# anassinator/pddp

Hardware: AMD Instinct MI355X
Metric: pddp_iterations_per_sec (higher is better)
Workload: dtype f32; 1 GPU; BASELINE.json configs[1]: cartpole n=4 m=1, known-dynamics iLQR, horizon=100, batch=4096 trajectories per GPU, bounds +-10 (eig-clamp + BoxQP branch), 10 line-search alphas; batch_per_gpu=4096, horizon=100, alphas=10, launch_form=10 rounds per launch, rounds_per_launch=10, backward_kernel_variant=0

## Files before the change

pddp_amd/csrc/accept.hpp:

```cpp
#pragma once

#include "pddp_common.hpp"

namespace pddp {

template <typename T>
struct AcceptArgs {
  int B, N, n, m, A;
  const T* Zc;
  const T* Uc;
  const T* Jc;
  const T* gains;
  const int32_t* bwd_status;
  double tol, max_reg;
  int n_iterations;
  T* Z;
  T* U;
  T* gains_acc;
  T* J_opt;
  double* mu;
  double* delta;
  int32_t* state;
  int32_t* iter;
  uint8_t* active;
  uint8_t* fresh;
  int32_t* n_live;
};

constexpr double kMuMin = 1e-6;
constexpr double kDelta0 = 2.0;

constexpr int kAcceptThreads = 64;
constexpr int kMaxAlphas = 16;
constexpr int kLiveShards = 256;


template <typename T>
struct AcceptIn {
  int bstat, iter;
  double mu, delta;
  T J_opt;
};
template <typename T>
PDDP_DEV AcceptIn<T> accept_load(const AcceptArgs<T>& a, int b) {
  AcceptIn<T> in;
  in.bstat = a.bwd_status[b];
  in.mu = a.mu[b];
  in.delta = a.delta[b];
  in.J_opt = a.J_opt[b];
  in.iter = a.iter[b];
  return in;
}

template <typename T>
PDDP_DEV int argmin_first(const T* J, int A, T& Jm_out) {
  int amin = 0;
  T Jm = J[0];
#pragma unroll
  for (int i = 1; i < kMaxAlphas; ++i) {
    const bool take = (i < A) && (Jm == Jm) && (J[i] < Jm || J[i] != J[i]);
    amin = take ? i : amin;
    Jm = take ? J[i] : Jm;
  }
  Jm_out = Jm;
  return amin;
}

template <typename T>
PDDP_DEV int accept_decide(const AcceptArgs<T>& a, int b, const AcceptIn<T>& in,
                           int amin, T J_new, bool& fresh_out) {
  int amin_out = -1;
  double mu = in.mu, delta = in.delta;
  int st;
  bool increase = false;
  if (in.bstat != 0) {
    increase = true;
    st = PDDP_STATE_NOT_PD;
  } else {
    const T J_opt = in.J_opt;
    if (J_new < J_opt) {
      amin_out = amin;
      delta = (delta < 1.0 ? delta : 1.0) / kDelta0;
      mu *= delta;
      if (mu <= kMuMin) mu = 0.0;
      const T rel = abs_(J_opt - J_new) / J_opt;
      st = (rel < (T)a.tol) ? PDDP_STATE_CONVERGED : PDDP_STATE_ACCEPTED;
      a.J_opt[b] = J_new;
    } else {
      increase = true;
      st = PDDP_STATE_REJECTED;
    }
  }
  if (increase) {
    delta = (delta > 1.0 ? delta : 1.0) * kDelta0;
    mu = (kMuMin > mu * delta) ? kMuMin : mu * delta;
    if (mu >= a.max_reg) st = PDDP_STATE_MAX_REG;
  }
  a.mu[b] = mu;
  a.delta[b] = delta;
  a.state[b] = st;
  uint8_t act = 0, fr = 0;
  if (st == PDDP_STATE_NOT_PD || st == PDDP_STATE_REJECTED) {
    act = 1;
  } else if (st == PDDP_STATE_ACCEPTED) {
    if (in.iter < a.n_iterations) {
      a.iter[b] = in.iter + 1;
      act = 1;
      fr = 1;
    }
  }
  a.active[b] = act;
  a.fresh[b] = fr;
  if (act && a.n_live != nullptr)
    atomicAdd(a.n_live + (b & (kLiveShards - 1)), 1);
  fresh_out = fr != 0;
  return amin_out;
}

}
```

pddp_amd/csrc/line_search_lds.hpp:

```cpp
#pragma once

#include <type_traits>
#include "models.hpp"
#include "problem_args.hpp"
#include "accept.hpp"
#include "riccati_n4.hpp"

namespace pddp {

template <typename T>
PDDP_DEV void group_copy(T* dst, const T* src, int count, int l16) {
  constexpr int kDeep = 8;
  for (int o0 = l16; o0 < count; o0 += 16 * kDeep) {
    T tmp[kDeep];
#pragma unroll
    for (int r = 0; r < kDeep; ++r) {
      const int o = o0 + 16 * r;
      tmp[r] = src[o < count ? o : 0];
    }
#pragma unroll
    for (int r = 0; r < kDeep; ++r) {
      const int o = o0 + 16 * r;
      if (o < count) dst[o] = tmp[r];
    }
  }
}

PDDP_DEV void store4(float* p, float a, float b, float c, float d) {
  *reinterpret_cast<float4*>(p) = make_float4(a, b, c, d);
}
PDDP_DEV void store4(double* p, double a, double b, double c, double d) {
  *reinterpret_cast<double2*>(p) = make_double2(a, b);
  *reinterpret_cast<double2*>(p + 2) = make_double2(c, d);
}

template <typename T, int n, int m>
PDDP_DEV void control_law(const T* z, const T* zr, const T* gr, const T* us,
                          T alpha, const T* umin, const T* umax, T* un) {
#pragma unroll
  for (int r = 0; r < m; ++r) {
    T s = T(0);
#pragma unroll
    for (int c = 0; c < n; ++c)
      s = n4::fma_(z[c] - zr[c], gr[m + r * n + c], s);
    const T du = n4::fma_(alpha, gr[r], s);
    const T v = us[r] + du;
    un[r] = clamp_nan(v, umin[r], umax[r]);
  }
}
PDDP_DEV float control_law_pk(f32x2 za, f32x2 zb, f32x2 zra, f32x2 zrb,
                              f32x2 g01, f32x2 g23, f32x2 g4u, float alpha,
                              float umin, float umax) {
  const f32x2 da = pk_sub(za, zra), db = pk_sub(zb, zrb);
  float s = n4::fma_(da.x, g01.y, 0.0f);
  s = n4::fma_(da.y, g23.x, s);
  s = n4::fma_(db.x, g23.y, s);
  s = n4::fma_(db.y, g4u.x, s);
  const float du = n4::fma_(alpha, g01.x, s);
  return clamp_nan(g4u.y + du, umin, umax);
}

#ifdef PDDP_WG_TIMELINE
__device__ long long g_search_timeline[1024][12];
#define PDDP_TLS(I)                                                           \
  do {                                                                        \
    if ((threadIdx.x & 255) == 0 && blockIdx.x < 1024)                        \
      g_search_timeline[blockIdx.x][(I) + 4 * (threadIdx.x >> 8)] =           \
          wall_clock64();                                                     \
  } while (0)
#define PDDP_TLS_AT(SLOT)                                                     \
  do {                                                                        \
    if (threadIdx.x == 0 && blockIdx.x < 1024)                                \
      g_search_timeline[blockIdx.x][SLOT] = wall_clock64();                   \
  } while (0)
#else
#define PDDP_TLS(I)
#define PDDP_TLS_AT(SLOT)
#endif

template <typename T>
struct PreStaged {
  const T* Zs;
  const T* Us;
  const T* Gs;
  int status;
  T J_opt;
  T* carry_rows = nullptr;
};
template <typename T, int MODEL, bool FUSED, int WPB, int H, unsigned QM,
          bool DENSE, bool PRE = false>
PDDP_DEV void line_search_lds_body(const ProblemT<T> P,
                                   const LineSearchArgs<T> a,
                                   const AcceptArgs<T> c, T* rec, T* Lout,
                                   unsigned char* smem_raw,
                                   const PreStaged<T> pre,
                                   const unsigned tid = threadIdx.x) {
  using D = ModelDims<MODEL>;
  constexpr int n = D::n, m = D::m;
  constexpr int GS = m + m * n;
  static_assert(H == 1 || (H == 2 && FUSED), "");
  static_assert(!DENSE || (FUSED && H == 1), "");
  static_assert(!PRE || (FUSED && H == 2 && !DENSE), "");
  constexpr int GST = PRE ? GS + m : GS;
  constexpr int UST = PRE ? GS + m : m;
  constexpr int kTailRows = DENSE ? 8 : 4;
  constexpr bool kPaired = PRE && MODEL == PDDP_MODEL_CARTPOLE &&
                           std::is_same<T, float>::value && GST == 6 &&
                           QM == kSparseMask<PDDP_MODEL_CARTPOLE>;
  __shared__ int sh_dec[WPB][4][2];
  const int lane = tid & (kWave - 1);
  const int wave_all = tid >> 6;
  const int wave = H == 1 ? wave_all : wave_all % WPB;
  const int hid = H == 1 ? 0 : wave_all / WPB;
  const int grp = lane >> 4, ai = lane & 15;
  const int N = a.N;
  const int per = DENSE ? N * GS : (N + 1) * n + N * m + N * GS;
  T* smem = reinterpret_cast<T*>(smem_raw) + (size_t)wave * 4 * per;
  const int b0 = (blockIdx.x * WPB + wave) * 4;
  PDDP_TLS(0);

  for (int g = 0; g < (PRE ? 0 : 4); ++g) {
    const int bg = b0 + g;
    if (bg >= a.B) break;
    if (H == 2 && (g & 1) != hid) continue;
    if (a.active != nullptr && a.active[bg] == 0) continue;
    T* dst = smem + (size_t)g * per;
    const T* zs = a.Z + (size_t)bg * (N + 1) * n;
    const T* us = a.U + (size_t)bg * N * m;
    const T* gs = a.gains + (size_t)bg * N * GS;
    if constexpr (DENSE) {
      for (int o = lane; o < N * GS; o += kWave) dst[o] = gs[o];
    } else {
      for (int o = lane; o < (N + 1) * n; o += kWave) dst[o] = zs[o];
      for (int o = lane; o < N * m; o += kWave) dst[(N + 1) * n + o] = us[o];
      for (int o = lane; o < N * GS; o += kWave)
        dst[(N + 1) * n + N * m + o] = gs[o];
    }
  }
  if constexpr (!PRE) __syncthreads();
  PDDP_TLS(1);

  const int b = b0 + grp;
  const bool exists = b < a.B;
  const int bc = exists ? b : a.B - 1;
  const bool attempted =
      exists && (a.active == nullptr || a.active[bc] != 0);
  const bool run =
      attempted && ai < a.A &&
      (PRE ? pre.status == 0
           : (a.bwd_status == nullptr || a.bwd_status[bc] == 0));
  if constexpr (!FUSED) {
    if (!run) return;
  }
  const bool bounded = a.u_min != nullptr && a.u_max != nullptr;
  T umin[m], umax[m];
#pragma unroll
  for (int r = 0; r < m; ++r) {
    umin[r] = bounded ? a.u_min[r] : -(T)__builtin_inff();
    umax[r] = bounded ? a.u_max[r] : (T)__builtin_inff();
  }
  const T* Zs = PRE ? pre.Zs
                    : DENSE ? a.Z + (size_t)bc * (N + 1) * n
                            : smem + (size_t)grp * per;
  const T* Us = PRE ? pre.Us
                    : DENSE ? a.U + (size_t)bc * N * m : Zs + (N + 1) * n;
  const T* Gs = PRE ? pre.Gs : DENSE ? smem + (size_t)grp * per : Us + N * m;
  const size_t zstep_c = (size_t)a.A * n, ustep_c = (size_t)a.A * m;
  AcceptIn<T> acc_in = {};
  if constexpr (FUSED) {
    if (attempted && ai == 0) {
      acc_in = accept_load(c, b);
      if constexpr (PRE) {
        acc_in.bstat = pre.status;
        acc_in.J_opt = pre.J_opt;
      }
    }
  }
  T Jmine = T(0);
  const bool nocand = FUSED && n <= 4 && Lout == nullptr && rec != nullptr &&
                      a.drop_candidates != 0 && N + 1 <= 16 * H * kTailRows;
  const bool store_uc = !(FUSED && n <= 6 && Lout == nullptr &&
                          rec != nullptr && N + 1 <= 16 * H * kTailRows);
  auto rollout = [&](T alpha, T* Zci, size_t zstep, T* Uci, size_t ustep,
                     auto cost) {
    if constexpr (kPaired) {
      typedef float V4_ __attribute__((ext_vector_type(4)));
      V4_ z4 = {Zs[0], Zs[1], Zs[2], Zs[3]};
      float J = 0.0f;
      auto step = [&](const int t) {
        const V4_ zr = *reinterpret_cast<const V4_*>(
            __builtin_assume_aligned(Zs + t * 4, 16));
        const f32x2* g2 = reinterpret_cast<const f32x2*>(
            __builtin_assume_aligned(Gs + t * 6, 8));
        const f32x2 g01 = g2[0], g23 = g2[1], g4u = g2[2];
        const f32x2 sc = sincos_pk(z4.z);
        __builtin_amdgcn_sched_barrier(0);
        __builtin_amdgcn_s_waitcnt(0xC07F);
        const float u = control_law_pk(z4.xy, z4.zw, zr.xy, zr.zw, g01, g23,
                                       g4u, alpha, umin[0], umax[0]);
#pragma unroll
        for (int j = 0; j < 4; ++j) Zci[(size_t)t * zstep + j] = z4[j];
        J += cartpole_cost_pk(P, z4.xy, sc, u);
        if constexpr (decltype(cost)::value) asm("" : "+v"(J));
        f32x2 na, nb;
        cartpole_dynamics_pk(P, z4.xy, z4.zw, sc, u, na, nb);
        z4 = V4_{na.x, na.y, nb.x, nb.y};
      };
      int t = 0;
      for (; t + 3 < N; t += 4) {
        step(t);
        step(t + 1);
        step(t + 2);
        step(t + 3);
      }
#pragma unroll 1
      for (; t < N; ++t) step(t);
      T z[n] = {z4.x, z4.y, z4.z, z4.w};
#pragma unroll
      for (int j = 0; j < n; ++j) Zci[(size_t)N * zstep + j] = z[j];
      const T lf =
          cost_value<T, MODEL>(P, z, nullptr, trig_of<T, MODEL>(z), true);
      return J + lf;
    }
    T z[n], zn[n], un[m];
#pragma unroll
    for (int j = 0; j < n; ++j) z[j] = Zs[j];
    T J = T(0);
    auto step = [&](const int t) {
      T zr[n], gr[GS], us[m];
      if constexpr (PRE && n == 4) {
        typedef T V4_ __attribute__((ext_vector_type(4)));
        const V4_ v = *reinterpret_cast<const V4_*>(
            __builtin_assume_aligned(Zs + t * 4, 16));
        zr[0] = v[0]; zr[1] = v[1]; zr[2] = v[2]; zr[3] = v[3];
      } else {
#pragma unroll
        for (int j = 0; j < n; ++j) zr[j] = Zs[t * n + j];
      }
      if constexpr (PRE && GST == 6) {
        typedef T V2_ __attribute__((ext_vector_type(2)));
        const V2_* g2 = reinterpret_cast<const V2_*>(
            __builtin_assume_aligned(Gs + t * 6, 8));
        const V2_ a0 = g2[0], a1 = g2[1], a2 = g2[2];
        gr[0] = a0[0]; gr[1] = a0[1]; gr[2] = a1[0]; gr[3] = a1[1];
        gr[4] = a2[0]; us[0] = a2[1];
      } else {
#pragma unroll
        for (int j = 0; j < GS; ++j) gr[j] = Gs[t * GST + j];
#pragma unroll
        for (int j = 0; j < m; ++j) us[j] = Us[t * UST + j];
      }
      const Trig<T, MODEL> tr = trig_of<T, MODEL>(z);
      __builtin_amdgcn_sched_barrier(0);
      if constexpr (PRE) __builtin_amdgcn_s_waitcnt(0xC07F);
      control_law<T, n, m>(z, zr, gr, us, alpha, umin, umax, un);
#pragma unroll
      for (int j = 0; j < n; ++j) Zci[(size_t)t * zstep + j] = z[j];
      if constexpr (!PRE) {
        if (store_uc) {
#pragma unroll
          for (int j = 0; j < m; ++j) Uci[(size_t)t * ustep + j] = un[j];
        }
      }
      J += cost_value<T, MODEL, QM>(P, z, un, tr, false);
      dynamics<T, MODEL, false>(P, z, un, tr, zn, nullptr, nullptr);
#pragma unroll
      for (int j = 0; j < n; ++j) z[j] = zn[j];
    };
    int t = 0;
    if constexpr (n <= 4) {
      for (; t + 3 < N; t += 4) {
        step(t);
        step(t + 1);
        step(t + 2);
        step(t + 3);
      }
    }
#pragma unroll 1
    for (; t < N; ++t) step(t);
#pragma unroll
    for (int j = 0; j < n; ++j) Zci[(size_t)N * zstep + j] = z[j];
    const T lf =
        cost_value<T, MODEL>(P, z, nullptr, trig_of<T, MODEL>(z), true);
    return J + lf;
  };
  if (run && hid == 0) {
    const T alpha = a.alphas[ai];
    const int idx = b * a.A + ai;
    const bool compact0 = FUSED && Lout == nullptr && rec != nullptr &&
                          ai == 0 && n <= 6 && N + 1 <= 16 * H * kTailRows;
    T* Zci = compact0 ? rec + (size_t)b * (N + 1) * n
                      : a.Zc + ((size_t)b * (N + 1) * a.A + ai) * n;
    T* Uci = a.Uc + ((size_t)b * N * a.A + ai) * m;
    const size_t zstep = compact0 ? (size_t)n : (nocand ? 0 : zstep_c);
    const size_t ustep = nocand ? 0 : ustep_c;
    Jmine = rollout(alpha, Zci, zstep, Uci, ustep, std::true_type{});
    a.Jc[idx] = Jmine;
  }
  PDDP_TLS(2);

  if constexpr (FUSED) {
    constexpr int kNone = 99;
    const T kInf = (T)__builtin_inff();
    const int nan_first =
        n4::group_min((run && Jmine != Jmine) ? ai : kNone);
    T Jf = (run && Jmine == Jmine) ? Jmine : kInf;
    {
      T y = n4::dpp<0x128>(Jf); Jf = y < Jf ? y : Jf;
      y = n4::dpp<0x12C>(Jf); Jf = y < Jf ? y : Jf;
      y = n4::dpp<(2 | (3 << 2) | (0 << 4) | (1 << 6))>(Jf); Jf = y < Jf ? y : Jf;
      y = n4::dpp<(1 | (0 << 2) | (3 << 4) | (2 << 6))>(Jf); Jf = y < Jf ? y : Jf;
    }
    const int min_first = n4::group_min((run && Jmine == Jf) ? ai : kNone);
    const int amin =
        nan_first != kNone ? nan_first : (min_first != kNone ? min_first : 0);
    const T J_new = nan_first != kNone ? (T)__builtin_nanf("") : Jf;

    int amin_out = -1, fresh_i = 0;
    if (attempted && ai == 0 && hid == 0) {
      bool fr;
      amin_out = accept_decide(c, b, acc_in, amin, J_new, fr);
      fresh_i = fr ? 1 : 0;
    }
    amin_out = __shfl(amin_out, lane & 48);
    fresh_i = __shfl(fresh_i, lane & 48);
    PDDP_TLS_AT(8);
    if constexpr (n <= 4) {
      if (nocand && hid == 0 && __any(amin_out > 0)) {
        if (amin_out > 0 && ai == amin_out)
          rollout(a.alphas[ai], rec + (size_t)b * (N + 1) * n, (size_t)n,
                  a.Uc + ((size_t)b * N * a.A + ai) * m, 0, std::false_type{});
      }
    }
    if constexpr (H == 1) {
      if (!__any(amin_out >= 0)) return;
      __builtin_amdgcn_fence(__ATOMIC_ACQ_REL, "workgroup");
    } else {
      if (hid == 0 && ai == 0) {
        sh_dec[wave][grp][0] = amin_out;
        sh_dec[wave][grp][1] = fresh_i;
      }
      __builtin_amdgcn_fence(__ATOMIC_ACQ_REL, "workgroup");
      __syncthreads();
      amin_out = sh_dec[wave][grp][0];
      fresh_i = sh_dec[wave][grp][1];
    }
    PDDP_TLS_AT(9);
    if (amin_out >= 0) {
      constexpr RecLayout lay(n, m);
      constexpr int S = lay.stride;
      const T* srcz = a.Zc + ((size_t)b * (N + 1) * a.A + amin_out) * n;
      const T* srcu = a.Uc + ((size_t)b * N * a.A + amin_out) * m;
      T* Zb = c.Z + (size_t)b * (N + 1) * n;
      T* Ub = c.U + (size_t)b * N * m;
      T* rec_b = rec + (size_t)b * (N + 1) * S;
      T* Ls = PRE ? nullptr : smem + (size_t)grp * per;
      const T* G = c.gains + (size_t)b * N * GS;
      T* Ga = c.gains_acc + (size_t)b * N * GS;
      T zc[n], uc[m];
      const int t_first = ai + 16 * hid;
      constexpr int KR = kTailRows;
      if (n <= 6 && Lout == nullptr && N + 1 <= 16 * H * KR) {
        T zz[KR][n], uu[KR][m];
        const bool from_rec = rec != nullptr && (amin_out == 0 || nocand);
        const T* cz = from_rec ? rec + (size_t)b * (N + 1) * n : srcz;
        const size_t czs = from_rec ? (size_t)n : zstep_c;
#pragma unroll
        for (int k = 0; k < KR; ++k) {
          const int t = t_first + 16 * H * k;
          const int tz = t <= N ? t : N;
#pragma unroll
          for (int j = 0; j < n; ++j) zz[k][j] = cz[(size_t)tz * czs + j];
        }
        const T* Gl = Gs;
        if constexpr (PRE) {
          for (int t = ai + 16 * hid; t < N; t += 16 * H) {
#pragma unroll
            for (int j = 0; j < GS; ++j) Ga[t * GS + j] = Gl[t * GST + j];
          }
        } else {
          constexpr int kDeep = 8;
          int o = ai + 16 * hid;
          for (; o + 16 * H * (kDeep - 1) < N * GS; o += 16 * H * kDeep) {
            T tmp[kDeep];
#pragma unroll
            for (int r = 0; r < kDeep; ++r) tmp[r] = Gl[o + 16 * H * r];
#pragma unroll
            for (int r = 0; r < kDeep; ++r) Ga[o + 16 * H * r] = tmp[r];
          }
          for (; o < N * GS; o += 16 * H) Ga[o] = Gl[o];
        }
        PDDP_TLS_AT(10);
        const T alpha_w = a.alphas[amin_out];
#pragma unroll
        for (int k = 0; k < KR; ++k) {
          const int t = t_first + 16 * H * k;
          const int tu = t < N ? t : 0;
          if constexpr (kPaired) {
            typedef float V4_ __attribute__((ext_vector_type(4)));
            const V4_ zr = *reinterpret_cast<const V4_*>(
                __builtin_assume_aligned(Zs + tu * 4, 16));
            const f32x2* g2 = reinterpret_cast<const f32x2*>(
                __builtin_assume_aligned(Gs + tu * 6, 8));
            uu[k][0] = control_law_pk(f32x2{zz[k][0], zz[k][1]},
                                      f32x2{zz[k][2], zz[k][3]}, zr.xy, zr.zw,
                                      g2[0], g2[1], g2[2], alpha_w, umin[0],
                                      umax[0]);
            continue;
          }
          T zr[n], gr[GS], us[m];
#pragma unroll
          for (int j = 0; j < n; ++j) zr[j] = Zs[tu * n + j];
#pragma unroll
          for (int j = 0; j < GS; ++j) gr[j] = Gs[tu * GST + j];
#pragma unroll
          for (int j = 0; j < m; ++j) us[j] = Us[tu * UST + j];
          control_law<T, n, m>(zz[k], zr, gr, us, alpha_w, umin, umax, uu[k]);
        }
#pragma unroll
        for (int k = 0; k < KR; ++k) {
          const int t = t_first + 16 * H * k;
          if (t <= N) {
#pragma unroll
            for (int j = 0; j < n; ++j) Zb[t * n + j] = zz[k][j];
          }
          if (t < N) {
#pragma unroll
            for (int j = 0; j < m; ++j) Ub[t * m + j] = uu[k][j];
          }
          if constexpr (PRE) {
            if (pre.carry_rows != nullptr && t <= N && N - t <= 16) {
              T* cr = pre.carry_rows + (N - t) * (n + m);
#pragma unroll
              for (int j = 0; j < n; ++j) cr[j] = zz[k][j];
              if (t < N) {
#pragma unroll
                for (int j = 0; j < m; ++j) cr[n + j] = uu[k][j];
              }
            }
          }
        }
      } else {
      {
        const int tz = t_first <= N ? t_first : N;
        const int tu = t_first < N ? t_first : 0;
#pragma unroll
        for (int j = 0; j < n; ++j) zc[j] = srcz[(size_t)tz * zstep_c + j];
#pragma unroll
        for (int j = 0; j < m; ++j) uc[j] = srcu[(size_t)tu * ustep_c + j];
      }
#pragma unroll 1
      for (int t = t_first; t <= N; t += 16 * H) {
        T zn_[n], un_[m];
        {
          const int t2 = t + 16 * H;
          const int tz = t2 <= N ? t2 : N, tu = t2 < N ? t2 : 0;
#pragma unroll
          for (int j = 0; j < n; ++j) zn_[j] = srcz[(size_t)tz * zstep_c + j];
#pragma unroll
          for (int j = 0; j < m; ++j) un_[j] = srcu[(size_t)tu * ustep_c + j];
        }
        const bool terminal = (t == N);
        T un[m];
#pragma unroll
        for (int j = 0; j < m; ++j) un[j] = terminal ? T(0) : uc[j];
#pragma unroll
        for (int j = 0; j < n; ++j) Zb[t * n + j] = zc[j];
        if (!terminal) {
#pragma unroll
          for (int j = 0; j < m; ++j) Ub[t * m + j] = un[j];
        }
        if (fresh_i && Lout != nullptr) {
          T w[S];
          const T l = record_of<T, MODEL>(P, zc, un, terminal, bounded, a.u_min,
                                         a.u_max, w);
          T* dst = rec_b + (size_t)t * S;
#pragma unroll
          for (int j = 0; j < S; j += 4)
            store4(dst + j, w[j], w[j + 1], w[j + 2], w[j + 3]);
          Lout[(size_t)b * (N + 1) + t] = l;
          Ls[t] = l;
        }
#pragma unroll
        for (int j = 0; j < n; ++j) zc[j] = zn_[j];
#pragma unroll
        for (int j = 0; j < m; ++j) uc[j] = un_[j];
      }
      if constexpr (H == 1) {
        group_copy(Ga, G, N * GS, ai);
      } else {
        const int half = (N * GS + 1) / 2;
        const int off = hid * half;
        const int cnt = hid == 0 ? half : N * GS - half;
        group_copy(Ga + off, G + off, cnt, ai);
      }
      }
      if constexpr (H == 1) {
        if (fresh_i && Lout != nullptr) {
          __builtin_amdgcn_fence(__ATOMIC_RELEASE, "wavefront");
          __builtin_amdgcn_wave_barrier();
          if (ai == 0) {
            T Jacc = T(0);
            for (int t = 0; t <= N; ++t) Jacc += Ls[t];
            c.J_opt[b] = Jacc;
            c.fresh[b] = 0;
          }
        }
      }
    }
    if constexpr (H == 2) {
      __syncthreads();
      if (!PRE && amin_out >= 0 && fresh_i && Lout != nullptr && hid == 0 &&
          ai == 0) {
        const T* Ls = smem + (size_t)grp * per;
        T Jacc = T(0);
        for (int t = 0; t <= N; ++t) Jacc += Ls[t];
        c.J_opt[b] = Jacc;
        c.fresh[b] = 0;
      }
    }
  }
  PDDP_TLS(3);
// ... 19 lines not shown
```

pddp_amd/csrc/riccati_n4_elem.hpp:

```cpp
#pragma once

#include <type_traits>
#include "models.hpp"
#include "riccati_n4_quad.hpp"

namespace pddp {

namespace n4d {
typedef float f32x4 __attribute__((ext_vector_type(4)));
PDDP_DEV int sgn(float x) { return __float_as_int(x); }
PDDP_DEV int splat(int w) {
  int r;
  asm("v_ashrrev_i32 %0, 31, %1" : "=v"(r) : "v"(w));
  return r;
}
PDDP_DEV float bsel(int mask, float a, float b) {
  float r;
  asm("v_bfi_b32 %0, %1, %2, %3" : "=v"(r) : "v"(mask), "v"(a), "v"(b));
  return r;
}

template <typename T>
struct GenArgs {
  const T* Z;
  const T* U;
  T* L;
  T* J_opt;
  uint8_t* fresh;
};
}

namespace n4e {

using n4::bperm;
using n4::dpp;
using n4::fma_;
using n4::group_sum;
using n4::kGain;
using n4::mul_nc;
using n4d::bsel;
using n4d::f32x4;
typedef float f32x2 __attribute__((ext_vector_type(2)));
typedef float f32x3 __attribute__((ext_vector_type(3)));
using n4d::GenArgs;
using n4d::sgn;
using n4d::splat;

constexpr int kWaves = 4;
constexpr int kTrajW = 4;
constexpr int kBlk = 16;
constexpr int kImg = 52;
constexpr int kRowStride = kBlk * kImg + 16;
constexpr int kImgBuf = kTrajW * kRowStride;
constexpr int kTermRow = 24;
constexpr int kTermSh = kTrajW * kTermRow;
constexpr int kPairLdsInl = kImgBuf;
constexpr int kPairLdsOvl = 2 * kImgBuf + kTermSh;

struct LsTableF {
  float v[n4::kLsSteps];
  constexpr LsTableF() : v() {
    for (int n = 0; n < n4::kLsSteps; ++n) v[n] = (float)n4::kLs.v[n];
  }
};
__device__ constexpr LsTableF kLsF{};
template <typename T>
PDDP_DEV const T* ls_table();
template <>
PDDP_DEV const float* ls_table<float>() { return kLsF.v; }
template <>
PDDP_DEV const double* ls_table<double>() { return n4::kLs.v; }
template <typename T>
struct Vec {
  typedef T v4 __attribute__((ext_vector_type(4)));
  typedef T v2 __attribute__((ext_vector_type(2)));
};

PDDP_DEV f32x2 lo_word(float a) {
  f32x2 r;
  r.x = a;
  return r;
}
PDDP_DEV f32x2 box_gaps(f32x2 lh, float x) {
  f32x2 d;
  asm("v_pk_add_f32 %0, %1, %2 op_sel_hi:[1,0] neg_lo:[0,1] neg_hi:[1,0]"
      : "=v"(d)
// ... 239 lines not shown
    } else {
      oddm = alive_m;
    }
    bool fail = false;
    if (__builtin_expect(oddm != 0, F32 ? 0 : 1)) {
      const bool take = (oddm & lane_bit) != 0;
      n4::QpClosed<T, true> qc;
      qc.solve(take ? kprev : T(0), take ? Quug : T(1), take ? Qu : T(0), lo_b,
               hi_b);
      T kx = qc.x;
      bool Kzero = !qc.free_;
      fail = qc.fail & take;
      const bool slow = qc.slow & take;
      if (__builtin_expect(__any(slow), 0)) {
        unsigned long long todo = __ballot(slow && l == 0);
        while (todo != 0) {
          const int src = __builtin_ctzll(todo);
          todo &= todo - 1;
          const n4::SlowQpOut<T> o = n4q::boxqp1_wave<T, true>(
              __shfl(kprev, src), __shfl(Quug, src), __shfl(Qu, src),
              __shfl(lo_b, src), __shfl(hi_b, src), ls_table<T>(), lane);
          const bool mine = (lane >> 4) == (src >> 4);
          kx = mine ? o.x : kx;
          Kzero = mine ? ((o.result_free & 1) == 0) : Kzero;
          fail = mine ? (o.result_free < 2) : fail;
        }
      }
      kt = take ? kx : kt;
      sK = take ? (Kzero ? T(0) : qc.inv) : sK;
    }
    if (fail) st = PDDP_BWD_BOXQP_FAILED;
  }
  return st;
}

#ifdef PDDP_ELEM_MARKS
__device__ long long g_elem_marks[8];
#define PDDP_EM_MARK(I) do { if (blockIdx.x == 0 && threadIdx.x == 0) g_elem_marks[I] = clock64(); } while (0)
#define PDDP_EM_ACC(I, T0) do { if (blockIdx.x == 0 && threadIdx.x == 0) g_elem_marks[I] += clock64() - (T0); } while (0)
#define PDDP_EM_NOW() clock64()
#else
#define PDDP_EM_MARK(I)
#define PDDP_EM_ACC(I, T0)
#define PDDP_EM_NOW() 0
#endif

#ifdef PDDP_WG_TIMELINE
__device__ long long g_elem_timeline[1024][12];
#define PDDP_TL(I)                                                            \
  do {                                                                        \
    if ((threadIdx.x & 255) == 0 && blockIdx.x < 1024)                        \
      g_elem_timeline[blockIdx.x][(I) + 4 * (threadIdx.x >> 8)] =             \
          wall_clock64();                                                     \
  } while (0)
#define PDDP_TL_HW(I)                                                         \
  do {                                                                        \
    if (threadIdx.x == 0 && blockIdx.x < 1024) {                              \
      g_elem_timeline[blockIdx.x][8] =                                        \
          __builtin_amdgcn_s_getreg(4 | (0 << 6) | (31 << 11));               \
      g_elem_timeline[blockIdx.x][9] =                                        \
          __builtin_amdgcn_s_getreg(20 | (0 << 6) | (3 << 11));               \
      g_elem_timeline[blockIdx.x][I] = clock64();                             \
    }                                                                         \
  } while (0)
#else
#define PDDP_TL(I)
#define PDDP_TL_HW(I)
#endif

struct RoundOut {
  const float* Zs;
  const float* Gs;
  const float* Us;
  int status;
  float J_opt;
  float* carry_rows;
};
constexpr int round_zu_stride(int N) { return 4 * (N + 1); }
constexpr int kCarryRows = kBlk + 1, kCarryW = 5;
constexpr int kCarryF = kTrajW * kCarryRows * kCarryW;
constexpr int kGainL = kGain + 1;
constexpr int round_gains_floats(int N) { return (kTrajW * N * kGainL + 3) & ~3; }

template <typename T, unsigned QM, bool OVL, bool ROUND, int BR = kBrEigBox>
PDDP_DEV bool elem_sweep_body(const RiccatiArgs<T>& a, const GenArgs<T>& gen,
                              const ProblemT<T>& prob, unsigned char* smem_raw,
                              RoundOut& ro,
                              const unsigned tid = threadIdx.x,
                              const int carry = -1) {
  static_assert(OVL || !ROUND, "");
  constexpr bool F32 = std::is_same<T, float>::value;
  static_assert(F32 || (!OVL && !ROUND), "");
  using V4 = typename Vec<T>::v4;
  using V2 = typename Vec<T>::v2;
  constexpr int MODEL = PDDP_MODEL_CARTPOLE;
  constexpr RecLayout lay(4, 1);
  constexpr bool BOUNDED = br_bounded(BR), CHOL = br_chol(BR);
  const int kPairLds = OVL ? kPairLdsOvl + (ROUND ? round_gains_floats(a.N) +
                                                        (carry >= 0 ? kCarryF : 0)
                                                  : 0)
                           : kPairLdsInl;
  const int lane = tid & (kWave - 1);
  const int wave = __builtin_amdgcn_readfirstlane((int)tid >> 6);
  const int pair = OVL ? (wave & (kWaves - 1)) : wave;
  const bool is_gen = OVL && wave >= kWaves;
  T* const img0 = reinterpret_cast<T*>(smem_raw) + pair * kPairLds;
  T* const term_w = OVL ? img0 + 2 * kImgBuf : img0;

  const int row = lane >> 4, l = lane & 15, i = l >> 2, j = l & 3;
  const int N = a.N;
  const int b0 = (blockIdx.x * kWaves + pair) * kTrajW;
  const int b = b0 + row;
  const bool exists = b < a.B;
  const int bc = exists ? b : a.B - 1;
  const T* Zg = gen.Z + (size_t)bc * (size_t)(N + 1) * 4;
  const T* Ug = gen.U + (size_t)bc * (size_t)N;
  const int nblk = (N + kBlk - 1) / kBlk;
  if (b0 >= a.B) return false;
  const bool counted = exists && (a.active == nullptr || a.active[bc] != 0);
  if (!__any(counted)) return false;
  PDDP_EM_MARK(0);
  PDDP_TL(0);
  PDDP_TL_HW(10);
  T umin = T(0), umax = T(0);
  if constexpr (BOUNDED) { umin = a.u_min[0]; umax = a.u_max[0]; }
  const int rbase = row * kRowStride;

  T zq[4], uq, Jacc = T(0), l_term = T(0);
  [[maybe_unused]] T* const carry_w =
      img0 + kPairLdsOvl + (ROUND ? round_gains_floats(N) : 0) +
      row * kCarryRows * kCarryW;
  if constexpr (ROUND) ro.carry_rows = carry >= 0 ? carry_w : nullptr;
  auto request = [&](int jb) {
    int tau = N - 1 - kBlk * jb - l;
    tau = tau < 0 ? 0 : tau;
    if constexpr (ROUND) {
      if (jb == 0 && carry == 0) {
        const T* cr = carry_w + (N - tau) * kCarryW;
        zq[0] = cr[0]; zq[1] = cr[1]; zq[2] = cr[2]; zq[3] = cr[3];
        uq = cr[4];
        return;
      }
    }
    const V4 v = *reinterpret_cast<const V4*>(Zg + 4 * tau);
    zq[0] = v[0]; zq[1] = v[1]; zq[2] = v[2]; zq[3] = v[3];
    uq = Ug[tau];
    if constexpr (ROUND) {
      if (jb == 0 && carry == 1 && N - tau <= kBlk) {
        T* cr = carry_w + (N - tau) * kCarryW;
        cr[0] = zq[0]; cr[1] = zq[1]; cr[2] = zq[2]; cr[3] = zq[3];
        cr[4] = uq;
      }
    }
  };
  auto terminal = [&]() {
    T zN[4];
    if (ROUND && carry == 0) {
      zN[0] = carry_w[0]; zN[1] = carry_w[1]; zN[2] = carry_w[2];
      zN[3] = carry_w[3];
    } else {
      const V4 zNv = *reinterpret_cast<const V4*>(Zg + 4 * N);
      zN[0] = zNv[0]; zN[1] = zNv[1]; zN[2] = zNv[2]; zN[3] = zNv[3];
      if (ROUND && carry == 1 && l == 0) {
        carry_w[0] = zN[0]; carry_w[1] = zN[1]; carry_w[2] = zN[2];
        carry_w[3] = zN[3];
      }
    }
    T lz[4], lzz[16], lu[1], luu[1];
    l_term = cost_derivs<T, MODEL>(prob, zN, nullptr, trig_of<T, MODEL>(zN),
                                   true, lz, lzz, lu, luu);
    T* scr = term_w + row * kTermRow;
    if (l == 0) {
#pragma unroll
      for (int k = 0; k < 16; k += 4)
        *reinterpret_cast<V4*>(scr + k) =
            V4{lzz[k], lzz[k + 1], lzz[k + 2], lzz[k + 3]};
      *reinterpret_cast<V4*>(scr + 16) = V4{lz[0], lz[1], lz[2], lz[3]};
      scr[20] = l_term;
      if (counted) gen.L[(size_t)bc * (size_t)(N + 1) + N] = l_term;
    }
  };
  auto pass = [&](int jb, T* buf) {
    const T z[4] = {zq[0], zq[1], zq[2], zq[3]};
    const T u = uq;
    if (jb + 1 < nblk) request(jb + 1);
    const int tau = N - 1 - kBlk * jb - l;
    T w[lay.stride];
    const T lc = record_of<T, MODEL, QM>(prob, z, &u, false, BOUNDED, a.u_min,
                                         a.u_max, w);
    T* dst = buf + rbase + l * kImg;
#pragma unroll
    for (int r = 0; r < 4; ++r)
      *reinterpret_cast<V4*>(dst + 4 * r) =
          V4{w[lay.oFz + ((r + 0) & 3) * 4 + r],
                w[lay.oFz + ((r + 1) & 3) * 4 + r],
                w[lay.oFz + ((r + 2) & 3) * 4 + r],
                w[lay.oFz + ((r + 3) & 3) * 4 + r]};
#pragma unroll
    for (int x = 0; x < 4; x += 2) {
      *reinterpret_cast<V4*>(dst + 16 + 2 * x) =
          V4{w[lay.oFu + x], w[lay.oLuz + x], w[lay.oFu + x + 1],
                w[lay.oLuz + x + 1]};
      *reinterpret_cast<V4*>(dst + 24 + 2 * x) =
          V4{w[lay.oFu + x], w[lay.oLz + x], w[lay.oFu + x + 1],
                w[lay.oLz + x + 1]};
    }
#pragma unroll
    for (int r = 0; r < 4; ++r)
      *reinterpret_cast<V4*>(dst + 32 + 4 * r) =
          V4{w[lay.oLzz + 4 * r], w[lay.oLzz + 4 * r + 1],
                w[lay.oLzz + 4 * r + 2], w[lay.oLzz + 4 * r + 3]};
    *reinterpret_cast<V4*>(dst + 48) =
        V4{w[lay.oLuu], w[lay.oLu], BOUNDED ? umin - w[lay.oU] : T(0),
           BOUNDED ? umax - w[lay.oU] : T(0)};
    if (tau >= 0) {
      if (counted) gen.L[(size_t)bc * (size_t)(N + 1) + tau] = lc;
      Jacc += lc;
    }
  };
  auto finish_costs = [&]() {
    const bool sums = counted && (gen.fresh == nullptr || gen.fresh[bc] != 0);
    const T Jrow = group_sum(Jacc) + (OVL ? term_w[row * kTermRow + 20] : l_term);
    if constexpr (ROUND) {
      const T Jold = gen.J_opt[bc];
      if (l == 0) term_w[row * kTermRow + 21] = sums ? Jrow : Jold;
    }
    if (sums && l == 0) {
      gen.J_opt[bc] = Jrow;
      if (gen.fresh != nullptr) gen.fresh[bc] = 0;
    }
  };
  [[maybe_unused]] T* const gains_w = img0 + kPairLdsOvl;
  auto flush_gains = [&](const T* ib, int t_top, int cnt) {
    const T* sg = ib + l * kImg + rbase;
    const V4 Kv = *reinterpret_cast<const V4*>(sg);
    const T kv = sg[4];
    if ((BR == kBrEigBox ? exists : counted) && l < cnt) {
      T* g = a.gains + ((size_t)bc * (size_t)N + (size_t)(t_top - l)) * kGain;
      g[0] = kv; g[1] = Kv[0]; g[2] = Kv[1]; g[3] = Kv[2]; g[4] = Kv[3];
      if constexpr (ROUND) {
        T* gl = gains_w + (row * N + (t_top - l)) * kGainL;
        gl[0] = kv; gl[1] = Kv[0]; gl[2] = Kv[1]; gl[3] = Kv[2]; gl[4] = Kv[3];
      }
    }
  };
  [[maybe_unused]] T* const zu_w =
      img0 + (nblk & 1) * kImgBuf + row * round_zu_stride(N);
  [[maybe_unused]] auto round_out = [&](int status_) {
    if constexpr (ROUND) {
      ro.Zs = zu_w;
      ro.Gs = gains_w + row * N * kGainL;
      ro.Us = ro.Gs + kGain;
      ro.status = status_;
      n4::lds_publish_barrier();
      ro.J_opt = term_w[row * kTermRow + 21];
    }
  };
  if constexpr (OVL) {
    if (is_gen) {
      request(0);
      pass(0, img0);
      PDDP_TL(1);
      n4::lds_publish_barrier();
      for (int jb = 1; jb < nblk; ++jb) {
        if (jb >= 2)
          flush_gains(img0 + (jb & 1) * kImgBuf, N - 1 - kBlk * (jb - 2), kBlk);
        pass(jb, img0 + (jb & 1) * kImgBuf);
        n4::lds_publish_barrier();
      }
      if (nblk >= 2)
        flush_gains(img0 + (nblk & 1) * kImgBuf, N - 1 - kBlk * (nblk - 2), kBlk);
      if constexpr (ROUND) {
        asm volatile("s_waitcnt lgkmcnt(0)" ::: "memory");
        constexpr int kCh = 8;
        V4 zc[kCh];
        T uc[kCh];
#pragma unroll
        for (int c = 0; c < kCh; ++c) {
          const int tz = l + 16 * c;
          zc[c] = *reinterpret_cast<const V4*>(Zg + 4 * (tz <= N ? tz : N));
          uc[c] = Ug[tz < N ? tz : 0];
        }
#pragma unroll
        for (int c = 0; c < kCh; ++c) {
          const int tz = l + 16 * c;
          if (tz <= N) *reinterpret_cast<V4*>(zu_w + 4 * tz) = zc[c];
          if (tz < N) gains_w[(row * N + tz) * kGainL + kGain] = uc[c];
        }
      }
      finish_costs();
      PDDP_TL(3);
      if constexpr (ROUND) round_out(PDDP_BWD_OK);
      return true;
    }
  }

  const T reg = (T)a.reg[bc];
  const int oA = rbase + 4 * i, oB = rbase + 4 * j, oL = rbase + 32 + l;
  const int oTi = rbase + 16 + 2 * i, oTj = rbase + 24 + 2 * j;
  const int tr_addr = ((lane & 48) | (j * 4 + i)) * 4;
  if constexpr (OVL) {
    __builtin_amdgcn_s_setprio(3);
    terminal();
    n4::lds_publish_barrier();
  } else {
    request(0);
    terminal();
    asm volatile("s_waitcnt lgkmcnt(0)" ::: "memory");
  }
  T V = term_w[row * kTermRow + l];
  T vc = term_w[row * kTermRow + 16 + j];

  struct Words {
    V4 Fs, Fq;
    V2 Ti, Tj;
    V4 Sc;
    T Lzz;
  };
  auto gather = [&](const T* ib, const int s) {
    const T* p = ib + s * kImg;
    Words w;
    w.Fs = *reinterpret_cast<const V4*>(p + oA);
    w.Fq = *reinterpret_cast<const V4*>(p + oB);
    w.Ti = *reinterpret_cast<const V2*>(p + oTi);
    w.Tj = *reinterpret_cast<const V2*>(p + oTj);
    w.Lzz = p[oL];
    w.Sc = *reinterpret_cast<const V4*>(p + 48 + rbase);
    return w;
  };
  T kprev = T(0);
  int status = PDDP_BWD_OK;
  unsigned long long alive_m = __ballot(counted);
  const int ostage = rbase + l;

  auto step = [&](const Words& w, T* ib, const int s) {
    const StepCoreT<T> q = step_core(V, vc, w.Ti[0], w.Tj[0], w.Fs, w.Fq,
                                     w.Lzz, w.Tj[1], w.Ti[1], w.Sc[0], w.Sc[1]);
    const T Quu = q.Quu, Qu = q.Qu;
    const T QzzT = bperm(tr_addr, q.Qzz);
    const T Quzc = bperm(tr_addr, q.Quzr);
    if constexpr (BR != kBrEigBox) {
      T Quug = Quu, Rr = q.Quzr, Rc = Quzc;
      if constexpr (CHOL) {
        const T fr = w.Ti[0], fc = w.Tj[0];
        const T ff = n4::dot_cols(fc, fc);
        T g = fr * w.Fs[0];
        g = fma_(n4::from_row_plus<1>(fr), w.Fs[1], g);
        g = fma_(n4::from_row_plus<2>(fr), w.Fs[2], g);
        g = fma_(n4::from_row_plus<3>(fr), w.Fs[3], g);
        Quug = fma_(reg, ff, Quu);
        Rr = fma_(reg, g, q.Quzr);
        Rc = bperm(tr_addr, Rr);
      }
      const bool alive = counted & (status == PDDP_BWD_OK);
      T kt, sK;
      int st = branch_gains<T, BR>(kprev, Quu, Qu, Quug, reg, w.Sc[2], w.Sc[3],
                                   alive, lane, kt, sK);
      const T Ks = -(sK * Rc);
      if constexpr (BR == kBrEig) {
        const bool nanK = n4::sum_cols((Ks != Ks) ? T(1) : T(0)) != T(0);
        if (nanK && st == PDDP_BWD_OK) st = PDDP_BWD_NAN;
      }
      status = (alive & (st != PDDP_BWD_OK)) ? st : status;
      ib[s * kImg + ostage] = (l < 4) ? Ks : kt;
      kprev = kt;
      const T sym = n4::opaque(q.Qzz + QzzT);
      if constexpr (CHOL) {
        const T wr = -(sK * fma_(Quu, kt, Qu));
        const T c2 = mul_nc(mul_nc(sK, sK), Quu);
        const T X = mul_nc(Rr, Quzc) + mul_nc(q.Quzr, Rc);
        V = fma_(T(0.5), sym, fma_(c2, mul_nc(Rr, Rc), -mul_nc(sK, X)));
        vc = fma_(kt, Quzc, fma_(wr, Rc, q.Qzc));
      } else {
        T c, wv;
        n4q::rank_one_coeffs(kt, sK, Quu, Qu, c, wv);
        V = fma_(T(0.5), sym, mul_nc(c, mul_nc(q.Quzr, Quzc)));
        vc = fma_(wv, Quzc, q.Qzc);
      }
      return;
    }
// ... 218 lines not shown
```

pddp_amd/csrc/round_n4_body.hpp:

```cpp
#pragma once

#include "riccati_n4_elem.hpp"
#include "line_search_lds.hpp"

namespace pddp {

template <unsigned QM, bool MULTI, int BR>
PDDP_DEV void round_n4_body(const RiccatiArgs<float>& a,
                            const n4d::GenArgs<float>& gen,
                            const ProblemT<float>& prob,
                            const LineSearchArgs<float>& ls,
                            const AcceptArgs<float>& ac, float* scratch,
                            int rounds, long long* phase_ticks, int use_carry) {
  extern __shared__ __attribute__((aligned(16))) unsigned char smem_raw[];
  const bool timed = phase_ticks != nullptr && threadIdx.x == 0;
  long long t_sweep = 0, t_search = 0;
  for (int r = 0;; ++r) {
    int z = 0;
    unsigned tid = threadIdx.x;
    if constexpr (MULTI) {
      asm volatile("s_mov_b32 %0, 0" : "=s"(z));
      asm volatile("" : "+v"(tid));
    }
    RiccatiArgs<float> a_r = a;
    a_r.N += z;
    LineSearchArgs<float> ls_r = ls;
    ls_r.N += z;
    AcceptArgs<float> ac_r = ac;
    ac_r.N += z;
    n4e::RoundOut ro;
    const long long t0 = timed ? wall_clock64() : 0;
    const int carry = MULTI && use_carry ? (r == 0 ? 1 : 0) : -1;
    if (!n4e::elem_sweep_body<float, QM, true, true, BR>(a_r, gen, prob,
                                                         smem_raw, ro, tid, carry))
      break;
    const long long t1 = timed ? wall_clock64() : 0;
    const PreStaged<float> pre{ro.Zs, ro.Us,      ro.Gs,
                               ro.status, ro.J_opt, ro.carry_rows};
    line_search_lds_body<float, PDDP_MODEL_CARTPOLE, true, n4e::kWaves, 2, QM,
                         false, true>(prob, ls_r, ac_r, scratch, nullptr,
                                      smem_raw, pre, tid);
    if (timed) {
      t_sweep += t1 - t0;
      t_search += wall_clock64() - t1;
    }
    if (!MULTI || r + 1 >= rounds) break;
    __builtin_amdgcn_fence(__ATOMIC_ACQ_REL, "workgroup");
    __syncthreads();
  }
  if (timed) {
    phase_ticks[2 * blockIdx.x] += t_sweep;
    phase_ticks[2 * blockIdx.x + 1] += t_search;
  }
}

int launch_round_n4_branches(const pddp_problem& p, const N4NominalPlan& pl,
                             const RiccatiArgs<float>& a,
                             const n4d::GenArgs<float>& gen,
                             const LineSearchArgs<float>& ls,
                             const AcceptArgs<float>& ac, float* scratch,
                             int rounds, long long* phase_ticks,
                             hipStream_t st);

}
```

Before: 50.31 million trajectory-iterations/s.

## Cache per-trajectory round state, alphas and bounds in LDS across fused rounds

In the multi-round fused kernel, per-trajectory accept state (mu, delta, J_opt, iter, active, fresh) is loaded once into shared memory and read from there in later rounds, instead of being reloaded from global arrays each round. Alphas and control bounds are also staged in LDS. The global writes are kept, so results still reach memory. It also removes the N-size guard so the compact tail path always runs under PRE, and reorders the gain copy to after the rollout. This adds more dependence on shared-state consistency, and the added asm barriers affect scheduling.

```diff
diff --git a/pddp_amd/csrc/accept.hpp b/pddp_amd/csrc/accept.hpp
--- a/pddp_amd/csrc/accept.hpp
+++ b/pddp_amd/csrc/accept.hpp
@@ -41,6 +41,16 @@
   double mu, delta;
   T J_opt;
 };
+
+struct RoundState {
+  double mu, delta;
+  float J_opt;
+  int32_t iter;
+  uint8_t active, fresh;
+  uint8_t pad_[6];
+};
+static_assert(sizeof(RoundState) == 32, "");
+
 template <typename T>
 PDDP_DEV AcceptIn<T> accept_load(const AcceptArgs<T>& a, int b) {
   AcceptIn<T> in;
@@ -49,6 +59,16 @@
   in.delta = a.delta[b];
   in.J_opt = a.J_opt[b];
   in.iter = a.iter[b];
+  return in;
+}
+template <typename T>
+PDDP_DEV AcceptIn<T> accept_load(const RoundState& rs) {
+  AcceptIn<T> in;
+  in.bstat = 0;
+  in.mu = rs.mu;
+  in.delta = rs.delta;
+  in.J_opt = (T)rs.J_opt;
+  in.iter = rs.iter;
   return in;
 }
 
@@ -66,9 +86,10 @@
   return amin;
 }
 
-template <typename T>
+template <typename T, bool REC = false>
 PDDP_DEV int accept_decide(const AcceptArgs<T>& a, int b, const AcceptIn<T>& in,
-                           int amin, T J_new, bool& fresh_out) {
+                           int amin, T J_new, bool& fresh_out,
+                           [[maybe_unused]] RoundState* rs = nullptr) {
   int amin_out = -1;
   double mu = in.mu, delta = in.delta;
   int st;
@@ -86,6 +107,7 @@
       const T rel = abs_(J_opt - J_new) / J_opt;
       st = (rel < (T)a.tol) ? PDDP_STATE_CONVERGED : PDDP_STATE_ACCEPTED;
       a.J_opt[b] = J_new;
+      if constexpr (REC) rs->J_opt = (float)J_new;
     } else {
       increase = true;
       st = PDDP_STATE_REJECTED;
@@ -105,12 +127,19 @@
   } else if (st == PDDP_STATE_ACCEPTED) {
     if (in.iter < a.n_iterations) {
       a.iter[b] = in.iter + 1;
+      if constexpr (REC) rs->iter = in.iter + 1;
       act = 1;
       fr = 1;
     }
   }
   a.active[b] = act;
   a.fresh[b] = fr;
+  if constexpr (REC) {
+    rs->mu = mu;
+    rs->delta = delta;
+    rs->active = act;
+    rs->fresh = fr;
+  }
   if (act && a.n_live != nullptr)
     atomicAdd(a.n_live + (b & (kLiveShards - 1)), 1);
   fresh_out = fr != 0;
diff --git a/pddp_amd/csrc/line_search_lds.hpp b/pddp_amd/csrc/line_search_lds.hpp
--- a/pddp_amd/csrc/line_search_lds.hpp
+++ b/pddp_amd/csrc/line_search_lds.hpp
@@ -88,19 +88,21 @@
   T* carry_rows = nullptr;
 };
 template <typename T, int MODEL, bool FUSED, int WPB, int H, unsigned QM,
-          bool DENSE, bool PRE = false>
+          bool DENSE, bool PRE = false, bool REC = false>
 PDDP_DEV void line_search_lds_body(const ProblemT<T> P,
                                    const LineSearchArgs<T> a,
                                    const AcceptArgs<T> c, T* rec, T* Lout,
                                    unsigned char* smem_raw,
                                    const PreStaged<T> pre,
-                                   const unsigned tid = threadIdx.x) {
+                                   const unsigned tid = threadIdx.x,
+                                   RoundState* rs_wg = nullptr) {
   using D = ModelDims<MODEL>;
   constexpr int n = D::n, m = D::m;
   constexpr int GS = m + m * n;
   static_assert(H == 1 || (H == 2 && FUSED), "");
   static_assert(!DENSE || (FUSED && H == 1), "");
   static_assert(!PRE || (FUSED && H == 2 && !DENSE), "");
+  static_assert(!REC || PRE, "");
   constexpr int GST = PRE ? GS + m : GS;
   constexpr int UST = PRE ? GS + m : m;
   constexpr int kTailRows = DENSE ? 8 : 4;
@@ -143,8 +145,17 @@
   const int b = b0 + grp;
   const bool exists = b < a.B;
   const int bc = exists ? b : a.B - 1;
-  const bool attempted =
-      exists && (a.active == nullptr || a.active[bc] != 0);
+  [[maybe_unused]] RoundState* rs = nullptr;
+  if constexpr (REC) {
+    unsigned t_rs = tid;
+    asm("" : "+v"(t_rs));
+    rs = rs_wg + ((t_rs >> 6) % WPB) * 4 + ((t_rs & (kWave - 1)) >> 4);
+  }
+  bool attempted;
+  if constexpr (REC)
+    attempted = exists && rs->active != 0;
+  else
+    attempted = exists && (a.active == nullptr || a.active[bc] != 0);
   const bool run =
       attempted && ai < a.A &&
       (PRE ? pre.status == 0
@@ -169,7 +180,10 @@
   AcceptIn<T> acc_in = {};
   if constexpr (FUSED) {
     if (attempted && ai == 0) {
-      acc_in = accept_load(c, b);
+      if constexpr (REC)
+        acc_in = accept_load<T>(*rs);
+      else
+        acc_in = accept_load(c, b);
       if constexpr (PRE) {
         acc_in.bstat = pre.status;
         acc_in.J_opt = pre.J_opt;
@@ -178,9 +192,11 @@
   }
   T Jmine = T(0);
   const bool nocand = FUSED && n <= 4 && Lout == nullptr && rec != nullptr &&
-                      a.drop_candidates != 0 && N + 1 <= 16 * H * kTailRows;
+                      a.drop_candidates != 0 &&
+                      (PRE || N + 1 <= 16 * H * kTailRows);
   const bool store_uc = !(FUSED && n <= 6 && Lout == nullptr &&
-                          rec != nullptr && N + 1 <= 16 * H * kTailRows);
+                          rec != nullptr &&
+                          (PRE || N + 1 <= 16 * H * kTailRows));
   auto rollout = [&](T alpha, T* Zci, size_t zstep, T* Uci, size_t ustep,
                      auto cost) {
     if constexpr (kPaired) {
@@ -288,7 +304,8 @@
     const T alpha = a.alphas[ai];
     const int idx = b * a.A + ai;
     const bool compact0 = FUSED && Lout == nullptr && rec != nullptr &&
-                          ai == 0 && n <= 6 && N + 1 <= 16 * H * kTailRows;
+                          ai == 0 && n <= 6 &&
+                          (PRE || N + 1 <= 16 * H * kTailRows);
     T* Zci = compact0 ? rec + (size_t)b * (N + 1) * n
                       : a.Zc + ((size_t)b * (N + 1) * a.A + ai) * n;
     T* Uci = a.Uc + ((size_t)b * N * a.A + ai) * m;
@@ -319,7 +336,7 @@
     int amin_out = -1, fresh_i = 0;
     if (attempted && ai == 0 && hid == 0) {
       bool fr;
-      amin_out = accept_decide(c, b, acc_in, amin, J_new, fr);
+      amin_out = accept_decide<T, REC>(c, b, acc_in, amin, J_new, fr, rs);
       fresh_i = fr ? 1 : 0;
     }
     amin_out = __shfl(amin_out, lane & 48);
@@ -327,6 +344,14 @@
     PDDP_TLS_AT(8);
     if constexpr (n <= 4) {
       if (nocand && hid == 0 && __any(amin_out > 0)) {
+        if constexpr (PRE) {
+          T alpha_r = a.alphas[ai];
+          asm volatile("" : "+v"(alpha_r));
+          if (amin_out > 0 && ai == amin_out)
+            rollout(alpha_r, rec + (size_t)b * (N + 1) * n, (size_t)n,
+                    a.Uc + ((size_t)b * N * a.A + ai) * m, 0,
+                    std::false_type{});
+        } else
         if (amin_out > 0 && ai == amin_out)
           rollout(a.alphas[ai], rec + (size_t)b * (N + 1) * n, (size_t)n,
                   a.Uc + ((size_t)b * N * a.A + ai) * m, 0, std::false_type{});
@@ -360,7 +385,7 @@
       T zc[n], uc[m];
       const int t_first = ai + 16 * hid;
       constexpr int KR = kTailRows;
-      if (n <= 6 && Lout == nullptr && N + 1 <= 16 * H * KR) {
+      if (n <= 6 && Lout == nullptr && (PRE || N + 1 <= 16 * H * KR)) {
         T zz[KR][n], uu[KR][m];
         const bool from_rec = rec != nullptr && (amin_out == 0 || nocand);
         const T* cz = from_rec ? rec + (size_t)b * (N + 1) * n : srcz;
@@ -374,10 +399,6 @@
         }
         const T* Gl = Gs;
         if constexpr (PRE) {
-          for (int t = ai + 16 * hid; t < N; t += 16 * H) {
-#pragma unroll
-            for (int j = 0; j < GS; ++j) Ga[t * GS + j] = Gl[t * GST + j];
-          }
         } else {
           constexpr int kDeep = 8;
           int o = ai + 16 * hid;
@@ -417,6 +438,13 @@
           for (int j = 0; j < m; ++j) us[j] = Us[tu * UST + j];
           control_law<T, n, m>(zz[k], zr, gr, us, alpha_w, umin, umax, uu[k]);
         }
+        if constexpr (PRE) {
+#pragma unroll
+          for (int k = 0; k < KR; ++k) {
+#pragma unroll
+            for (int j = 0; j < n; ++j) asm volatile("" : "+v"(zz[k][j]));
+          }
+        }
 #pragma unroll
         for (int k = 0; k < KR; ++k) {
           const int t = t_first + 16 * H * k;
@@ -438,6 +466,12 @@
                 for (int j = 0; j < m; ++j) cr[n + j] = uu[k][j];
               }
             }
+          }
+        }
+        if constexpr (PRE) {
+          for (int t = ai + 16 * hid; t < N; t += 16 * H) {
+#pragma unroll
+            for (int j = 0; j < GS; ++j) Ga[t * GS + j] = Gl[t * GST + j];
           }
         }
       } else {
diff --git a/pddp_amd/csrc/riccati_n4_elem.hpp b/pddp_amd/csrc/riccati_n4_elem.hpp
--- a/pddp_amd/csrc/riccati_n4_elem.hpp
+++ b/pddp_amd/csrc/riccati_n4_elem.hpp
@@ -2,6 +2,7 @@
 
 #include <type_traits>
 #include "models.hpp"
+#include "accept.hpp"
 #include "riccati_n4_quad.hpp"
 
 namespace pddp {
@@ -407,12 +408,15 @@
 constexpr int kGainL = kGain + 1;
 constexpr int round_gains_floats(int N) { return (kTrajW * N * kGainL + 3) & ~3; }
 
-template <typename T, unsigned QM, bool OVL, bool ROUND, int BR = kBrEigBox>
+template <typename T, unsigned QM, bool OVL, bool ROUND, int BR = kBrEigBox,
+          bool REC = false>
 PDDP_DEV bool elem_sweep_body(const RiccatiArgs<T>& a, const GenArgs<T>& gen,
                               const ProblemT<T>& prob, unsigned char* smem_raw,
                               RoundOut& ro,
                               const unsigned tid = threadIdx.x,
-                              const int carry = -1) {
+                              const int carry = -1,
+                              RoundState* rs_wg = nullptr) {
+  static_assert(ROUND || !REC, "");
   static_assert(OVL || !ROUND, "");
   constexpr bool F32 = std::is_same<T, float>::value;
   static_assert(F32 || (!OVL && !ROUND), "");
@@ -442,7 +446,13 @@
   const T* Ug = gen.U + (size_t)bc * (size_t)N;
   const int nblk = (N + kBlk - 1) / kBlk;
   if (b0 >= a.B) return false;
-  const bool counted = exists && (a.active == nullptr || a.active[bc] != 0);
+  [[maybe_unused]] RoundState* const rs =
+      REC ? rs_wg + pair * kTrajW + row : nullptr;
+  bool counted;
+  if constexpr (REC)
+    counted = exists && rs->active != 0;
+  else
+    counted = exists && (a.active == nullptr || a.active[bc] != 0);
   if (!__any(counted)) return false;
   PDDP_EM_MARK(0);
   PDDP_TL(0);
@@ -470,6 +480,11 @@
     const V4 v = *reinterpret_cast<const V4*>(Zg + 4 * tau);
     zq[0] = v[0]; zq[1] = v[1]; zq[2] = v[2]; zq[3] = v[3];
     uq = Ug[tau];
+    if constexpr (REC) {
+      if (jb == 0)
+        asm volatile("" : "+v"(zq[0]), "+v"(zq[1]), "+v"(zq[2]), "+v"(zq[3]),
+                          "+v"(uq));
+    }
     if constexpr (ROUND) {
       if (jb == 0 && carry == 1 && N - tau <= kBlk) {
         T* cr = carry_w + (N - tau) * kCarryW;
@@ -486,6 +501,8 @@
     } else {
       const V4 zNv = *reinterpret_cast<const V4*>(Zg + 4 * N);
       zN[0] = zNv[0]; zN[1] = zNv[1]; zN[2] = zNv[2]; zN[3] = zNv[3];
+      if constexpr (REC)
+        asm volatile("" : "+v"(zN[0]), "+v"(zN[1]), "+v"(zN[2]), "+v"(zN[3]));
       if (ROUND && carry == 1 && l == 0) {
         carry_w[0] = zN[0]; carry_w[1] = zN[1]; carry_w[2] = zN[2];
         carry_w[3] = zN[3];
@@ -544,15 +561,27 @@
     }
   };
   auto finish_costs = [&]() {
-    const bool sums = counted && (gen.fresh == nullptr || gen.fresh[bc] != 0);
+    bool sums;
+    if constexpr (REC)
+      sums = counted && rs->fresh != 0;
+    else
+      sums = counted && (gen.fresh == nullptr || gen.fresh[bc] != 0);
     const T Jrow = group_sum(Jacc) + (OVL ? term_w[row * kTermRow + 20] : l_term);
     if constexpr (ROUND) {
-      const T Jold = gen.J_opt[bc];
+      T Jold;
+      if constexpr (REC)
+        Jold = rs->J_opt;
+      else
+        Jold = gen.J_opt[bc];
       if (l == 0) term_w[row * kTermRow + 21] = sums ? Jrow : Jold;
     }
     if (sums && l == 0) {
       gen.J_opt[bc] = Jrow;
       if (gen.fresh != nullptr) gen.fresh[bc] = 0;
+      if constexpr (REC) {
+        rs->J_opt = Jrow;
+        rs->fresh = 0;
+      }
     }
   };
   [[maybe_unused]] T* const gains_w = img0 + kPairLdsOvl;
@@ -620,7 +649,11 @@
     }
   }
 
-  const T reg = (T)a.reg[bc];
+  T reg;
+  if constexpr (REC)
+    reg = (T)rs->mu;
+  else
+    reg = (T)a.reg[bc];
   const int oA = rbase + 4 * i, oB = rbase + 4 * j, oL = rbase + 32 + l;
   const int oTi = rbase + 16 + 2 * i, oTj = rbase + 24 + 2 * j;
   const int tr_addr = ((lane & 48) | (j * 4 + i)) * 4;
diff --git a/pddp_amd/csrc/round_n4_body.hpp b/pddp_amd/csrc/round_n4_body.hpp
--- a/pddp_amd/csrc/round_n4_body.hpp
+++ b/pddp_amd/csrc/round_n4_body.hpp
@@ -15,6 +15,45 @@
   extern __shared__ __attribute__((aligned(16))) unsigned char smem_raw[];
   const bool timed = phase_ticks != nullptr && threadIdx.x == 0;
   long long t_sweep = 0, t_search = 0;
+  [[maybe_unused]] RoundState* rs_wg = nullptr;
+  [[maybe_unused]] const float* ub = nullptr;
+  [[maybe_unused]] const float* alphas_l = nullptr;
+  constexpr bool kBounds = MULTI && n4e::br_bounded(BR);
+  if constexpr (kBounds) {
+    __shared__ float sh_ub[2];
+    const float lo = a.u_min[0], hi = a.u_max[0];
+    sh_ub[0] = lo;
+    sh_ub[1] = hi;
+    ub = sh_ub;
+  }
+  if constexpr (MULTI) {
+    __shared__ RoundState sh_rs[n4e::kWaves * n4e::kTrajW];
+    __shared__ float sh_alpha[kMaxAlphas];
+    rs_wg = sh_rs;
+    alphas_l = sh_alpha;
+    {
+      const int ai = threadIdx.x & (kMaxAlphas - 1);
+      sh_alpha[ai] = ls.alphas[ai < ls.A ? ai : ls.A - 1];
+    }
+    const int pair = (threadIdx.x >> 6) & (n4e::kWaves - 1);
+    const int row = (threadIdx.x & (kWave - 1)) >> 4;
+    const int b = (blockIdx.x * n4e::kWaves + pair) * n4e::kTrajW + row;
+    const int bc = b < ac.B ? b : ac.B - 1;
+    RoundState st;
+    st.mu = ac.mu[bc];
+    st.delta = ac.delta[bc];
+    st.J_opt = ac.J_opt[bc];
+    st.iter = ac.iter[bc];
+    st.active = ac.active[bc];
+    st.fresh = ac.fresh[bc];
+    RoundState* rs = sh_rs + pair * n4e::kTrajW + row;
+    rs->mu = st.mu;
+    rs->delta = st.delta;
+    rs->J_opt = st.J_opt;
+    rs->iter = st.iter;
+    rs->active = st.active;
+    rs->fresh = st.fresh;
+  }
   for (int r = 0;; ++r) {
     int z = 0;
     unsigned tid = threadIdx.x;
@@ -28,18 +67,24 @@
     ls_r.N += z;
     AcceptArgs<float> ac_r = ac;
     ac_r.N += z;
+    if constexpr (MULTI) ls_r.alphas = alphas_l;
+    if constexpr (kBounds) {
+      a_r.u_min = ls_r.u_min = ub;
+      a_r.u_max = ls_r.u_max = ub + 1;
+    }
     n4e::RoundOut ro;
     const long long t0 = timed ? wall_clock64() : 0;
     const int carry = MULTI && use_carry ? (r == 0 ? 1 : 0) : -1;
-    if (!n4e::elem_sweep_body<float, QM, true, true, BR>(a_r, gen, prob,
-                                                         smem_raw, ro, tid, carry))
+    if (!n4e::elem_sweep_body<float, QM, true, true, BR, MULTI>(
+            a_r, gen, prob, smem_raw, ro, tid, carry, rs_wg))
       break;
     const long long t1 = timed ? wall_clock64() : 0;
     const PreStaged<float> pre{ro.Zs, ro.Us,      ro.Gs,
                                ro.status, ro.J_opt, ro.carry_rows};
     line_search_lds_body<float, PDDP_MODEL_CARTPOLE, true, n4e::kWaves, 2, QM,
-                         false, true>(prob, ls_r, ac_r, scratch, nullptr,
-                                      smem_raw, pre, tid);
+                         false, true, MULTI>(prob, ls_r, ac_r, scratch,
+                                             nullptr, smem_raw, pre, tid,
+                                             rs_wg);
     if (timed) {
       t_sweep += t1 - t0;
       t_search += wall_clock64() - t1;
```

New measurement: 51.84 million trajectory-iterations/s (median of 6 runs). 1.03x the previous value.
